# lyclyc52/Instance_NeRF

Measured on AMD Instinct MI355X. Metric: Msamples/sec (train+infer) 3D-FRONT 800x800 at 1/2/4/8 MI355X; PSNR parity, higher is better.
Workload: dtype f32; 1 GPU; render 800x800 synthetic 3D-FRONT-like room, hash-grid NeRF L=16 F=2 T=6119864 sigma+rgb (BASELINE configs[1]), one view per step per GPU; parallelism=views sharded over 1 GPU(s), no data-path collective

## Files before the change

### instance_nerf_amd/csrc/field_fused.hip

```cpp
#include <atomic>
#include <mutex>
#include <type_traits>

#include "common.h"
#include "grid_common.h"

namespace inr {

typedef float f32x4 __attribute__((ext_vector_type(4)));
typedef __bf16 bf16x8 __attribute__((ext_vector_type(8)));

#ifndef INR_MLP_FP32
#define INR_MLP_FP32 0
#endif

#ifdef INR_PROBE_BUILD
#include "probe/field_probe.h"
#else
#if defined(INR_PROBE_MODE) || defined(INR_PROBE_STATIC) || defined(INR_PROBE_SLOW_XCD)
#error "INR_PROBE_* switches need -DINR_PROBE_BUILD (tools/build_probe.py): those variants produce wrong results"
#endif
#define INR_PROBE_PROLOGUE()
#define INR_PROBE_SCHEDULE(steal)
#define INR_PROBE_TILE()
// ... 250 lines not shown
    hi[t] = __uint_as_float(r0) + __uint_as_float(r1);
  }
}


template <int N_MT, int N_G>
__device__ __forceinline__ void layer(const float4* __restrict__ w, int lane, const f32x4* in, f32x4* out) {
  if constexpr (N_MT == 1) {
    f32x4 a0 = {0.f, 0.f, 0.f, 0.f}, a1 = {0.f, 0.f, 0.f, 0.f};
#pragma unroll
    for (int g = 0; g < N_G; g += 2) {
      __builtin_amdgcn_sched_barrier(0);
      const float4 w0 = w[g * 64 + lane], w1 = w[(g + 1) * 64 + lane];
      a0 = __builtin_amdgcn_mfma_f32_16x16x4f32(w0.x, in[g][0], a0, 0, 0, 0);
      a1 = __builtin_amdgcn_mfma_f32_16x16x4f32(w1.x, in[g + 1][0], a1, 0, 0, 0);
      a0 = __builtin_amdgcn_mfma_f32_16x16x4f32(w0.y, in[g][1], a0, 0, 0, 0);
      a1 = __builtin_amdgcn_mfma_f32_16x16x4f32(w1.y, in[g + 1][1], a1, 0, 0, 0);
      a0 = __builtin_amdgcn_mfma_f32_16x16x4f32(w0.z, in[g][2], a0, 0, 0, 0);
      a1 = __builtin_amdgcn_mfma_f32_16x16x4f32(w1.z, in[g + 1][2], a1, 0, 0, 0);
      a0 = __builtin_amdgcn_mfma_f32_16x16x4f32(w0.w, in[g][3], a0, 0, 0, 0);
      a1 = __builtin_amdgcn_mfma_f32_16x16x4f32(w1.w, in[g + 1][3], a1, 0, 0, 0);
    }
    out[0] = a0 + a1;
  } else {
    f32x4 acc[N_MT];
#pragma unroll
    for (int mt = 0; mt < N_MT; ++mt) acc[mt] = f32x4{0.f, 0.f, 0.f, 0.f};
#pragma unroll
    for (int g = 0; g < N_G; ++g) {
      __builtin_amdgcn_sched_barrier(0);
      float4 wv[N_MT];
#pragma unroll
      for (int mt = 0; mt < N_MT; ++mt) wv[mt] = w[(mt * N_G + g) * 64 + lane];
#pragma unroll
      for (int mt = 0; mt < N_MT; ++mt) acc[mt] = __builtin_amdgcn_mfma_f32_16x16x4f32(wv[mt].x, in[g][0], acc[mt], 0, 0, 0);
#pragma unroll
      for (int mt = 0; mt < N_MT; ++mt) acc[mt] = __builtin_amdgcn_mfma_f32_16x16x4f32(wv[mt].y, in[g][1], acc[mt], 0, 0, 0);
#pragma unroll
      for (int mt = 0; mt < N_MT; ++mt) acc[mt] = __builtin_amdgcn_mfma_f32_16x16x4f32(wv[mt].z, in[g][2], acc[mt], 0, 0, 0);
#pragma unroll
      for (int mt = 0; mt < N_MT; ++mt) acc[mt] = __builtin_amdgcn_mfma_f32_16x16x4f32(wv[mt].w, in[g][3], acc[mt], 0, 0, 0);
    }
#pragma unroll
    for (int mt = 0; mt < N_MT; ++mt) out[mt] = acc[mt];
  }
}

struct SplitB {
  uint4 hi, lo;
};

__device__ __forceinline__ void split2(float x0, float x1, uint32_t& hi, uint32_t& lo) {
  const uint32_t u0 = __float_as_uint(x0), u1 = __float_as_uint(x1);
  hi = __builtin_amdgcn_perm(u1, u0, 0x07060302u);
  const float l0 = x0 - __uint_as_float(u0 & 0xFFFF0000u);
  const float l1 = x1 - __uint_as_float(u1 & 0xFFFF0000u);
  lo = __builtin_amdgcn_perm(__float_as_uint(l1), __float_as_uint(l0), 0x07060302u);
}
__device__ __forceinline__ SplitB split8(const f32x4 a, const f32x4 b) {
  SplitB r;
  split2(a[0], a[1], r.hi.x, r.lo.x);
  split2(a[2], a[3], r.hi.y, r.lo.y);
  split2(b[0], b[1], r.hi.z, r.lo.z);
  split2(b[2], b[3], r.hi.w, r.lo.w);
  return r;
}
__device__ __forceinline__ f32x4 mfma_bf(const uint4 a, const uint4 b, const f32x4 c) {
  return __builtin_amdgcn_mfma_f32_16x16x32_bf16(__builtin_bit_cast(bf16x8, a), __builtin_bit_cast(bf16x8, b), c, 0, 0, 0);
}

template <int N_MT, int N_S>
__device__ __forceinline__ void layer_bf(const uint4* __restrict__ w, int lane, const SplitB* in, f32x4* out) {
  if constexpr (N_MT == 1) {
    f32x4 a0 = {0.f, 0.f, 0.f, 0.f}, a1 = a0, a2 = a0;
#pragma unroll
    for (int st = 0; st < N_S; ++st) {
      __builtin_amdgcn_sched_barrier(0);
      const uint4 wh = w[(st * 2 + 0) * 64 + lane], wlo = w[(st * 2 + 1) * 64 + lane];
      a0 = mfma_bf(wh, in[st].hi, a0);
      a1 = mfma_bf(wlo, in[st].hi, a1);
      a2 = mfma_bf(wh, in[st].lo, a2);
    }
    out[0] = a0 + (a1 + a2);
  } else {
    f32x4 acc[N_MT];
#pragma unroll
    for (int mt = 0; mt < N_MT; ++mt) acc[mt] = f32x4{0.f, 0.f, 0.f, 0.f};
#pragma unroll
    for (int st = 0; st < N_S; ++st) {
      __builtin_amdgcn_sched_barrier(0);
      uint4 wh[N_MT], wlo[N_MT];
#pragma unroll
      for (int mt = 0; mt < N_MT; ++mt) {
        wh[mt] = w[((mt * N_S + st) * 2 + 0) * 64 + lane];
        wlo[mt] = w[((mt * N_S + st) * 2 + 1) * 64 + lane];
      }
#pragma unroll
      for (int mt = 0; mt < N_MT; ++mt) acc[mt] = mfma_bf(wh[mt], in[st].hi, acc[mt]);
#pragma unroll
      for (int mt = 0; mt < N_MT; ++mt) acc[mt] = mfma_bf(wlo[mt], in[st].hi, acc[mt]);
#pragma unroll
      for (int mt = 0; mt < N_MT; ++mt) acc[mt] = mfma_bf(wh[mt], in[st].lo, acc[mt]);
    }
#pragma unroll
    for (int mt = 0; mt < N_MT; ++mt) out[mt] = acc[mt];
  }
}

typedef _Float16 f16x8_t __attribute__((ext_vector_type(8)));
typedef _Float16 f16x2_t __attribute__((ext_vector_type(2)));
typedef float f32x2_t __attribute__((ext_vector_type(2)));
__device__ __forceinline__ uint32_t pack_f16x2(float a, float b) {
  const f32x2_t v = {a, b};
  return __builtin_bit_cast(uint32_t, __builtin_convertvector(v, f16x2_t));
}
template <int N_MT, int N_S>
__device__ __forceinline__ void layer_h1(const uint4* __restrict__ w, int lane, const uint4* in, f32x4* out) {
  f32x4 acc[N_MT];
#pragma unroll
  for (int mt = 0; mt < N_MT; ++mt) acc[mt] = f32x4{0.f, 0.f, 0.f, 0.f};
#pragma unroll
  for (int st = 0; st < N_S; ++st) {
    __builtin_amdgcn_sched_barrier(0);
#pragma unroll
    for (int mt = 0; mt < N_MT; ++mt)
      acc[mt] = __builtin_amdgcn_mfma_f32_16x16x32_f16(__builtin_bit_cast(f16x8_t, w[((mt * N_S + st) * 2 + 0) * 64 + lane]),
                                                       __builtin_bit_cast(f16x8_t, in[st]), acc[mt], 0, 0, 0);
  }
#pragma unroll
  for (int mt = 0; mt < N_MT; ++mt) out[mt] = acc[mt];
}

template <int N_MT, int N_G, bool kFast = false>
__device__ __forceinline__ void mlp_layer(const float4* __restrict__ wsec, int lane, const f32x4* in, f32x4* out) {
#if INR_MLP_FP32
  layer<N_MT, N_G>(wsec, lane, in, out);
#else
  if constexpr (kFast) {
    uint4 b[N_G / 2];
#pragma unroll
    for (int st = 0; st < N_G / 2; ++st)
      b[st] = uint4{pack_f16x2(in[2 * st][0], in[2 * st][1]), pack_f16x2(in[2 * st][2], in[2 * st][3]),
                    pack_f16x2(in[2 * st + 1][0], in[2 * st + 1][1]), pack_f16x2(in[2 * st + 1][2], in[2 * st + 1][3])};
    layer_h1<N_MT, N_G / 2>(reinterpret_cast<const uint4*>(wsec), lane, b, out);
  } else {
    SplitB b[N_G / 2];
#pragma unroll
    for (int st = 0; st < N_G / 2; ++st) b[st] = split8(in[2 * st], in[2 * st + 1]);
    layer_bf<N_MT, N_G / 2>(reinterpret_cast<const uint4*>(wsec), lane, b, out);
  }
#endif
}

__device__ __forceinline__ float rgb_channel_of_lane(const f32x4 o) {
  const auto a = __builtin_amdgcn_permlane16_swap(__float_as_uint(o[0]), __float_as_uint(o[1]), false, false);
  const unsigned a0 = a[0];
  const auto b = __builtin_amdgcn_permlane32_swap(a0, __float_as_uint(o[2]), false, false);
  const unsigned b0 = b[0];
  return __uint_as_float(b0);
}
__device__ __forceinline__ float sigmoid_rgb(float o) {
  return __frcp_rn(1.0f + __expf(-o));
}

__device__ __forceinline__ float select4(int q, float a, float b, float c, float d) {
  return q == 0 ? a : (q == 1 ? b : (q == 2 ? c : d));
}

struct TileIn {
  float x0, x1, x2;
  float d0, d1, d2;
  bool oob;
};

__device__ __forceinline__ float to_x01(float x, float bound, float rb, float) { return (x + bound) / rb; }

template <bool kDir>
__device__ __forceinline__ void load_tile_in(const float* __restrict__ x, const float* __restrict__ d, int64_t m,
                                             float bound, float rb, float rb_inv, TileIn& t) {
  t.x0 = to_x01(x[m * 3 + 0], bound, rb, rb_inv);
  t.x1 = to_x01(x[m * 3 + 1], bound, rb, rb_inv);
  t.x2 = to_x01(x[m * 3 + 2], bound, rb, rb_inv);
  t.oob = oob01(t.x0, t.x1, t.x2);
  if (t.oob) t.x0 = t.x1 = t.x2 = 0.0f;
  if constexpr (kDir) {
    t.d0 = d[m * 3]; t.d1 = d[m * 3 + 1]; t.d2 = d[m * 3 + 2];
  }
}

constexpr int kXcdChunkLog2 = 10;
#ifndef INR_STEAL_SHIFT
#define INR_STEAL_SHIFT 1
#endif
constexpr int kStealRoundsShift = INR_STEAL_SHIFT;
struct TileSched {
  int64_t lo, hi;
  int64_t first;
  int64_t stride;
  int64_t main_local = 0, tail_base = 0;
  int64_t n_main = 0, tail = 0;
  int64_t static_local = 0;
  uint32_t xcd = 0;
  bool interleaved = false, hybrid = false;
  __device__ __forceinline__ int64_t tile_of(int y, int64_t u) const {
    if (u < main_local) return ((((u >> kXcdChunkLog2) << 3) + y) << kXcdChunkLog2) + (u & ((1 << kXcdChunkLog2) - 1));
    return n_main + tail * y / 8 + (u - main_local);
  }
  __device__ __forceinline__ int64_t local_end(int y) const { return main_local + tail * (y + 1) / 8 - tail * y / 8; }
  __device__ __forceinline__ int64_t tile(int64_t i) const {
    if (interleaved) {
      const int64_t u = first + i * stride;
      if (u < main_local)
        return ((((u >> kXcdChunkLog2) << 3) + xcd) << kXcdChunkLog2) + (u & ((1 << kXcdChunkLog2) - 1));
      return tail_base + (u - main_local);
    }
    return first + i * stride;
  }
};
__device__ __forceinline__ TileSched make_sched(int64_t n_tiles, int waves_per_block, bool steal = false) {
  const int nb = gridDim.x, b = blockIdx.x;
  const int w = threadIdx.x >> 6;
  TileSched s;
  if (nb % 8 == 0) {
    const int xcd = b & 7, local = b >> 3, per = nb >> 3;
    const int64_t rounds = n_tiles >> (kXcdChunkLog2 + 3);
    if (rounds >= 4) {
      const int64_t n_main = rounds << (kXcdChunkLog2 + 3), tail = n_tiles - n_main;
      s.interleaved = true;
      s.xcd = (uint32_t)xcd;
      s.main_local = rounds << kXcdChunkLog2;
      s.n_main = n_main;
      s.tail = tail;
      s.hybrid = steal;
      s.static_local = steal ? (rounds - max((int64_t)1, rounds >> kStealRoundsShift)) << kXcdChunkLog2 : s.main_local;
      s.tail_base = n_main + tail * xcd / 8;
      s.lo = 0;
      s.hi = n_main + tail * (xcd + 1) / 8;
      s.first = (int64_t)local * waves_per_block + w;
      s.stride = (int64_t)per * waves_per_block;
      return s;
    }
    s.lo = n_tiles * xcd / 8;
    s.hi = n_tiles * (xcd + 1) / 8;
    s.first = s.lo + (int64_t)local * waves_per_block + w;
    s.stride = (int64_t)per * waves_per_block;
  } else {
    s.lo = 0;
    s.hi = n_tiles;
    s.first = (int64_t)b * waves_per_block + w;
    s.stride = (int64_t)nb * waves_per_block;
  }
  return s;
}

constexpr int kFieldThreads = 512;
constexpr int kGroupChunkLog2 = 6;
constexpr int kGroupDraw = 1;
constexpr int kGroupPools = 4;
struct GroupDraw {
  unsigned long long* cursor;
  int owner, n_owner;
  __device__ __forceinline__ void init(unsigned long long* cursors, int pools) {
    const int n_xcd = (gridDim.x % 8 == 0) ? 8 : 1;
    const int n_pool = (gridDim.x % (8 * pools) == 0) ? pools : 1;
    const int xcd = (n_xcd == 8) ? (int)(blockIdx.x & 7) : 0;
    const int pool = (n_pool > 1) ? (int)((blockIdx.x >> 3) % pools) : 0;
    owner = pool * n_xcd + xcd;
    n_owner = n_pool * n_xcd;
    cursor = cursors + owner;
  }
  __device__ __forceinline__ int64_t group_of(uint32_t u) const {
    const int64_t chunk = (int64_t)(u >> kGroupChunkLog2) * n_owner + owner;
    return (chunk << kGroupChunkLog2) + (u & ((1u << kGroupChunkLog2) - 1u));
  }
  __device__ __forceinline__ int64_t draw() const { return group_of((uint32_t)atomicAdd(cursor, (unsigned long long)kGroupDraw)); }
};
constexpr int kStealPools = 4, kStealOwners = 8 * kStealPools, kStealDraw = 4, kStealBlockLog2 = 6;
struct TileWalk {
  TileSched s;
  unsigned long long* cur;
  int lane, own, owner, sub;
  int64_t it, k_base;
  unsigned long long raw_next;
  bool dyn;
  __device__ __forceinline__ void init(const TileSched& sched, unsigned long long* cursors) {
    s = sched; cur = cursors; lane = threadIdx.x & 63; it = 0; dyn = false; sub = kStealDraw; k_base = 0; raw_next = 0;
    own = owner = (int)(((blockIdx.x >> 3) % kStealPools) * 8 + (blockIdx.x & 7));
    if (!cursors) s.hybrid = false;
    if (!s.hybrid) s.static_local = s.main_local;
  }
  __device__ __forceinline__ int64_t pool_len(int o) const {
    const int64_t nb = (s.local_end(o & 7) - s.static_local + (1 << kStealBlockLog2) - 1) >> kStealBlockLog2;
    const int p = o >> 3;
    return nb > p ? ((nb - p + kStealPools - 1) / kStealPools) << kStealBlockLog2 : 0;
  }
  __device__ __forceinline__ int64_t local_of(int o, int64_t k) const {
    return s.static_local + ((((k >> kStealBlockLog2) * kStealPools) + (o >> 3)) << kStealBlockLog2) +
           (k & ((1 << kStealBlockLog2) - 1));
  }
  __device__ __forceinline__ unsigned long long issue(int o) const {
    unsigned long long v = 0;
    if (lane == 0) v = atomicAdd(cur + o, (unsigned long long)kStealDraw);
    return v;
  }
  __device__ __forceinline__ static int64_t uniform(unsigned long long v) {
    return (int64_t)(((unsigned long long)(uint32_t)__builtin_amdgcn_readfirstlane((int)(v >> 32)) << 32) |
                     (uint32_t)__builtin_amdgcn_readfirstlane((int)v));
  }
  __device__ __forceinline__ int scan() const {
    bool live = false;
    if (lane < kStealOwners) live = (int64_t)__hip_atomic_load(cur + lane, __ATOMIC_RELAXED, __HIP_MEMORY_SCOPE_AGENT) < pool_len(lane);
    const uint32_t mask = (uint32_t)__ballot(live);
    for (int i = 0; i < kStealOwners; ++i) {
      const int o = (((own >> 3) + i) % kStealPools) * 8 + (((own & 7) + i / kStealPools) & 7);
      if ((mask >> o) & 1u) return o;
    }
    return -1;
  }
  __device__ __forceinline__ int64_t next() {
    if (!dyn) {
      if (!s.hybrid) {
        const int64_t t = s.tile(it++);
        return t < s.hi ? t : -1;
      }
      const int64_t u = s.first + (it++) * s.stride;
      if (u < s.static_local) return s.tile_of((int)s.xcd, u);
      dyn = true;
      raw_next = issue(owner);
    }
    for (;;) {
      if (sub < kStealDraw) {
        const int64_t u = local_of(owner, k_base + sub);
        ++sub;
        if (u < s.local_end(owner & 7)) return s.tile_of(owner & 7, u);
        continue;
      }
      int64_t k = uniform(raw_next);
      while (k >= pool_len(owner)) {
        const int o = scan();
        if (o < 0) return -1;
        owner = o;
        k = uniform(issue(owner));
      }
      k_base = k;
      sub = 0;
      raw_next = issue(owner);
    }
  }
};
constexpr int kFieldMinWaves = 2;

__device__ __forceinline__ f32x4 load4(const float* p) {
  const float4 v = *reinterpret_cast<const float4*>(p);
  return f32x4{v.x, v.y, v.z, v.w};
}
__device__ __forceinline__ void store4(float* p, f32x4 v) {
  *reinterpret_cast<float4*>(p) = make_float4(v[0], v[1], v[2], v[3]);
}
__device__ __forceinline__ f32x4 mask4(f32x4 g, f32x4 h) {
  return f32x4{h[0] > 0.f ? g[0] : 0.f, h[1] > 0.f ? g[1] : 0.f, h[2] > 0.f ? g[2] : 0.f, h[3] > 0.f ? g[3] : 0.f};
}

struct NerfSave {
  float *enc, *h1, *so, *cin, *c1, *c2;
};

template <bool kColor, bool kTable = false, int kSave = 0, bool kHalf = false, bool kFast = false, bool kPre = false>
__global__ void __launch_bounds__(kFieldThreads, kFieldMinWaves) k_nerf_fwd(const float* __restrict__ x, const float* __restrict__ d,
                                                               int64_t M, const int32_t* __restrict__ n_dev, float bound,
                                                               const float2* __restrict__ emb, uint32_t emb_bytes, GridDesc G,
                                                               const float4* __restrict__ packed, float density_scale,
                                                               float* __restrict__ sigma, float* __restrict__ rgb,
                                                               float* __restrict__ geo, const int32_t* __restrict__ ray_ids,
                                                               const float4* __restrict__ shq, NerfSave sv,
                                                               unsigned long long* __restrict__ steal) {
  extern __shared__ __attribute__((aligned(16))) float4 wl[];
  INR_PROBE_PROLOGUE();
  __builtin_amdgcn_s_setprio(3);
  constexpr int kStage = (kColor ? kNerfFloats : kCol0) / 4;
  for (int i = threadIdx.x; i < kStage; i += kFieldThreads) wl[i] = packed[i];
  LevelRec* recs = reinterpret_cast<LevelRec*>(wl + kStage);
  stage_level_recs(G, recs);
  __syncthreads();

  constexpr int kWaves = kFieldThreads / 64;
  const int lane = threadIdx.x & 63, q = lane >> 4, j = lane & 15;
  int64_t n = M;
  if (n_dev) n = min((int64_t)*n_dev, M);
  const int64_t n_tiles = (n + 15) >> 4;
  const float rb = 2.0f * bound;
  const float rb_inv = 0.0f;
  INR_PROBE_SCHEDULE(steal);
  TileWalk walk;
  walk.init(make_sched(n_tiles, kWaves, steal != nullptr), steal);

  const bool all_hashed[4] = {slot_all_hashed(G, 0), slot_all_hashed(G, 1), slot_all_hashed(G, 2), slot_all_hashed(G, 3)};
  const __amdgpu_buffer_rsrc_t rsrc = __builtin_amdgcn_make_buffer_rsrc((void*)emb, 0, (int)emb_bytes, 0x00020000);

  for (int64_t tile = walk.next(); tile >= 0; tile = walk.next()) {
    INR_PROBE_TILE();
    const int64_t m = tile * 16 + j;
    const bool valid = m < n;
    TileIn me;
    f32x4 sh_in = {0.f, 0.f, 0.f, 0.f};
    if constexpr (kTable) {
      const int64_t mm = valid ? m : n - 1;
      me.x0 = x[mm * 3 + 0]; me.x1 = x[mm * 3 + 1]; me.x2 = x[mm * 3 + 2];
      const float4 t4 = shq[(int64_t)ray_ids[mm] * 4 + q];
      sh_in = f32x4{t4.x, t4.y, t4.z, t4.w};
    } else {
      load_tile_in<kColor>(x, d, valid ? m : n - 1, bound, rb, rb_inv, me);
    }

    f32x4 enc[2];
    {
      Gathered g;
      uint32_t rec_off = (uint32_t)q * 4u * (uint32_t)sizeof(LevelRec);
      asm volatile("" : "+v"(rec_off));
      typedef float v2f __attribute__((ext_vector_type(2)));
      v2f fine_a = {0.f, 0.f}, fine_b = {0.f, 0.f};
      if constexpr (kPre) {
        static_assert(!kPre || kTable, "the sliced feed is a variant of the table feed");
        static_assert(kSliceLevels == 3, "lane map below");
        const v2f* pre = reinterpret_cast<const v2f*>(d);
        const int64_t m_pad = (M + 31) & ~(int64_t)31, mm = valid ? m : n - 1;
        const int sl = (q & 1) ? 1 : 0;
        fine_a = __builtin_nontemporal_load(pre + (int64_t)sl * m_pad + mm);
        fine_b = __builtin_nontemporal_load(pre + (int64_t)(sl + 1) * m_pad + mm);
      }
      issue_gathers<kHalf, kPre>(reinterpret_cast<const LevelRec*>(reinterpret_cast<const char*>(recs) + rec_off), all_hashed,
                                 rsrc, me.x0, me.x1, me.x2, g);
      __builtin_amdgcn_sched_barrier(0);
      blend<kHalf>(g, enc[0], enc[1]);
      if constexpr (kPre) {
        if (q == 2) enc[1] = f32x4{enc[1][0], enc[1][1], fine_a.x, fine_a.y};
        else if (q == 3) enc[1] = f32x4{fine_a.x, fine_a.y, fine_b.x, fine_b.y};
      }
    }
    if constexpr (!kTable) {
      if (me.oob) enc[0] = enc[1] = f32x4{0.f, 0.f, 0.f, 0.f};
    }
    INR_PROBE_AFTER_GATHER();

    f32x4 h1[4];
    mlp_layer<4, 2, kFast>(wl + kSig0 / 4, lane, enc, h1);
#pragma unroll
    for (int t = 0; t < 4; ++t) h1[t] = relu4(h1[t]);
    f32x4 h2[1];
    mlp_layer<1, 4, kFast>(wl + kSig1 / 4, lane, h1, h2);

    if (valid) {
      if (q == 0) sigma[m] = __expf(h2[0][0]) * density_scale;
      if (INR_PROBE_GEO_IS_OUTPUT && geo) {
#pragma unroll
        for (int r = 0; r < 4; ++r) {
          const int row = 4 * q + r;
          if (row >= 1) geo[m * 15 + row - 1] = h2[0][r];
        }
      }
    }

    if constexpr (kColor) {
      f32x4 cin[2];
      if constexpr (kTable) {
        cin[0] = sh_in;
      } else {
        float sh[16];
        sh4(me.d0, me.d1, me.d2, sh);
#pragma unroll
        for (int ks = 0; ks < 4; ++ks) cin[0][ks] = select4(q, sh[4 * ks], sh[4 * ks + 1], sh[4 * ks + 2], sh[4 * ks + 3]);
      }
      cin[1] = h2[0];
      f32x4 c1[4], c2[4], o[1];
      mlp_layer<4, 2, kFast>(wl + kCol0 / 4, lane, cin, c1);
#pragma unroll
      for (int t = 0; t < 4; ++t) c1[t] = relu4(c1[t]);
      mlp_layer<4, 4, kFast>(wl + kCol1 / 4, lane, c1, c2);
#pragma unroll
      for (int t = 0; t < 4; ++t) c2[t] = relu4(c2[t]);
      mlp_layer<1, 4, kFast>(wl + kCol2 / 4, lane, c2, o);
      if constexpr (kSave == 2) {
        if (valid) {
#pragma unroll
          for (int t = 0; t < 2; ++t) store4(sv.enc + m * 32 + 16 * t + 4 * q, enc[t]);
        }
      }
      if constexpr (kSave == 1) {
        if (valid) {
#pragma unroll
          for (int t = 0; t < 2; ++t) store4(sv.enc + m * 32 + 16 * t + 4 * q, enc[t]);
          store4(sv.so + m * 16 + 4 * q, h2[0]);
#pragma unroll
          for (int t = 0; t < 4; ++t) {
            store4(sv.h1 + m * 64 + 16 * t + 4 * q, h1[t]);
            store4(sv.c1 + m * 64 + 16 * t + 4 * q, c1[t]);
            store4(sv.c2 + m * 64 + 16 * t + 4 * q, c2[t]);
          }
#pragma unroll
          for (int ks = 0; ks < 4; ++ks) sv.cin[m * 32 + 4 * ks + q] = cin[0][ks];
#pragma unroll
          for (int r = 0; r < 4; ++r) {
            const int row = 4 * q + r;
            sv.cin[m * 32 + (row >= 1 ? 15 + row : 31)] = row >= 1 ? h2[0][r] : 0.f;
          }
        }
      }
      const float ch = sigmoid_rgb(rgb_channel_of_lane(o[0]));
      if (valid && q < 3) rgb[m * 3 + q] = ch;
    }
  }
  INR_PROBE_EPILOGUE();
}

constexpr int kSliceThreads = 256;
constexpr int kSliceTilesPerIter = 4;
struct SliceX {
  float x0, x1, x2;
};
__device__ __forceinline__ SliceX slice_load_x(const float* __restrict__ x01, int64_t m, int64_t M) {
  const int64_t mm = m < M ? m : M - 1;
  const float* p = x01 + mm * 3;
  return SliceX{__builtin_nontemporal_load(p), __builtin_nontemporal_load(p + 1), __builtin_nontemporal_load(p + 2)};
}
__global__ void __launch_bounds__(kSliceThreads) k_grid_fine_slices(const float* __restrict__ x01, int64_t M,
                                                                    const float2* __restrict__ emb, uint32_t emb_bytes,
                                                                    GridDesc G, float* __restrict__ pre) {
  const int slice = blockIdx.y;
  const int l = 16 - kSliceLevels + slice;
  const float sc = G.scales[l];
  const uint32_t m_ = G.mask[l], res1 = G.res1[l];
  const bool h = m_ != 0;
  const uint32_t base = G.offsets[l] * 8u, pa = h ? 2654435761u : res1, pb = h ? 805459861u : res1 * res1;
  const uint32_t mask = h ? m_ : 0xFFFFFFFFu;
  const __amdgpu_buffer_rsrc_t rsrc = __builtin_amdgcn_make_buffer_rsrc((void*)emb, 0, (int)emb_bytes, 0x00020000);
  const int lane = threadIdx.x & 63, w = threadIdx.x >> 6;
  const uint32_t side = (uint32_t)(lane & 1);
  constexpr int kWaves = kSliceThreads / 64;
  constexpr int kT = kSliceTilesPerIter;
  const int64_t m_pad = (M + 31) & ~(int64_t)31;
  const int64_t n_iter = (M + 32 * kT - 1) / (32 * kT);
  float* __restrict__ out = pre + (int64_t)slice * m_pad * 2;
  for (int64_t it = (int64_t)blockIdx.x * kWaves + w; it < n_iter; it += (int64_t)gridDim.x * kWaves) {
    u32x2 rows[kT][4];
    float wx[kT], fy[kT], fz[kT];
#pragma unroll
    for (int t = 0; t < kT; ++t) {
      const SliceX X = slice_load_x(x01, (it * kT + t) * 32 + (lane >> 1), M);
      const float px = X.x0 * sc + 0.5f, py = X.x1 * sc + 0.5f, pz = X.x2 * sc + 0.5f;
      const float fx = __builtin_amdgcn_fractf(px);
      wx[t] = side ? fx : 1.0f - fx;
      fy[t] = __builtin_amdgcn_fractf(py); fz[t] = __builtin_amdgcn_fractf(pz);
      const uint32_t c = (uint32_t)px + side, cy = (uint32_t)py, cz = (uint32_t)pz;
      const uint32_t hy0 = cy * pa, hy1 = hy0 + pa;
      const uint32_t hz0 = cz * pb, hz1 = hz0 + pb;
      const uint32_t yz[4] = {h ? (hy0 ^ hz0) : (hy0 + hz0), h ? (hy1 ^ hz0) : (hy1 + hz0),
                              h ? (hy0 ^ hz1) : (hy0 + hz1), h ? (hy1 ^ hz1) : (hy1 + hz1)};
#pragma unroll
      for (int k = 0; k < 4; ++k) {
        const uint32_t idx = (h ? (c ^ yz[k]) : (c + yz[k])) & mask;
        rows[t][k] = gather_row<false>(rsrc, base + idx * 8u);
      }
    }
#pragma unroll
    for (int t = 0; t < kT; ++t) {
      const f32x2 wy = {1.0f - fy[t], fy[t]};
      const f32x2 xy = wy * wx[t];
      const f32x2 w0 = xy * (1.0f - fz[t]), w1 = xy * fz[t];
      f32x2 acc = {0.f, 0.f};
      acc = __builtin_elementwise_fma(w0.xx, row2<false>(rows[t][0]), acc);
      acc = __builtin_elementwise_fma(w0.yy, row2<false>(rows[t][1]), acc);
      acc = __builtin_elementwise_fma(w1.xx, row2<false>(rows[t][2]), acc);
      acc = __builtin_elementwise_fma(w1.yy, row2<false>(rows[t][3]), acc);
      const float ox = __shfl_xor(acc.x, 1), oy = __shfl_xor(acc.y, 1);
      const float v = side ? acc.y + oy : acc.x + ox;
      const int64_t m = (it * kT + t) * 32 + (lane >> 1);
      if (m < M) __builtin_nontemporal_store(v, out + m * 2 + side);
    }
  }
}

struct LatticeDesc {
  const float* ax_w;
  const float* ax_l;
  const float* ax_h;
  int W, L, H, Wp;
};
constexpr int kMaxExtractDirs = 8;
template <bool kLattice>
__global__ void __launch_bounds__(kFieldThreads, kFieldMinWaves) k_nerf_fwd_dirs(
    const float* __restrict__ x, int64_t M, float bound, const float2* __restrict__ emb, uint32_t emb_bytes, GridDesc G,
    const float4* __restrict__ packed, const float* __restrict__ sh_dirs , int D, float4* __restrict__ out,
    LatticeDesc lat, float logit_min) {
  extern __shared__ __attribute__((aligned(16))) float4 wl[];
  constexpr int kStage = kNerfFloats / 4;
  for (int i = threadIdx.x; i < kStage; i += kFieldThreads) wl[i] = packed[i];
  LevelRec* recs = reinterpret_cast<LevelRec*>(wl + kStage);
  stage_level_recs(G, recs);
  float* shl = reinterpret_cast<float*>(recs + 16);
  for (int i = threadIdx.x; i < D * 16; i += kFieldThreads) {
    const int d = i >> 4, qq = (i >> 2) & 3, ks = i & 3;
    shl[i] = sh_dirs[d * 16 + 4 * ks + qq];
  }
  __syncthreads();
  constexpr int kWaves = kFieldThreads / 64;
  const int lane = threadIdx.x & 63, q = lane >> 4, j = lane & 15;
  const int64_t n_tiles = (M + 15) >> 4;
  const float rb = 2.0f * bound;
  const TileSched sched = make_sched(n_tiles, kWaves);
  const bool all_hashed[4] = {slot_all_hashed(G, 0), slot_all_hashed(G, 1), slot_all_hashed(G, 2), slot_all_hashed(G, 3)};
  const __amdgpu_buffer_rsrc_t rsrc = __builtin_amdgcn_make_buffer_rsrc((void*)emb, 0, (int)emb_bytes, 0x00020000);
  const float inv_d = 1.0f / (float)D;
  for (int64_t it = 0, tile = sched.tile(0); tile < sched.hi; tile = sched.tile(++it)) {
    int64_t m = tile * 16 + j;
    bool valid = m < M;
    TileIn me;
    if constexpr (kLattice) {
      const int64_t row = m / lat.Wp;
      const int iw = (int)(m - row * lat.Wp);
      const int il = (int)(row / lat.H), ih = (int)(row - (int64_t)il * lat.H);
      valid = valid && iw < lat.W;
      const int cw = min(iw, lat.W - 1), cl = min(il, lat.L - 1);
      me.x0 = to_x01(fminf(fmaxf(lat.ax_w[cw], -bound), bound), bound, rb, 0.0f);
      me.x1 = to_x01(fminf(fmaxf(lat.ax_l[cl], -bound), bound), bound, rb, 0.0f);
      me.x2 = to_x01(fminf(fmaxf(lat.ax_h[ih], -bound), bound), bound, rb, 0.0f);
      me.oob = oob01(me.x0, me.x1, me.x2);
      if (me.oob) me.x0 = me.x1 = me.x2 = 0.0f;
      m = ((int64_t)cw * lat.L + cl) * lat.H + ih;
    } else {
      load_tile_in<false>(x, nullptr, valid ? m : M - 1, bound, rb, 0.0f, me);
    }
    f32x4 enc[2];
    {
      Gathered g;
      uint32_t rec_off = (uint32_t)q * 4u * (uint32_t)sizeof(LevelRec);
      asm volatile("" : "+v"(rec_off));
      issue_gathers(reinterpret_cast<const LevelRec*>(reinterpret_cast<const char*>(recs) + rec_off), all_hashed, rsrc,
                    me.x0, me.x1, me.x2, g);
      __builtin_amdgcn_sched_barrier(0);
      blend(g, enc[0], enc[1]);
    }
    if (me.oob) enc[0] = enc[1] = f32x4{0.f, 0.f, 0.f, 0.f};
    f32x4 h1[4], h2[1];
    mlp_layer<4, 2>(wl + kSig0 / 4, lane, enc, h1);
#pragma unroll
    for (int t = 0; t < 4; ++t) h1[t] = relu4(h1[t]);
    mlp_layer<1, 4>(wl + kSig1 / 4, lane, h1, h2);
    float ch = 0.f;
    for (int d = 0; d < D; ++d) {
      f32x4 cin[2], c1[4], c2[4], o[1];
      const float4 s4 = *reinterpret_cast<const float4*>(shl + d * 16 + q * 4);
      cin[0] = f32x4{s4.x, s4.y, s4.z, s4.w};
      cin[1] = h2[0];
      mlp_layer<4, 2>(wl + kCol0 / 4, lane, cin, c1);
#pragma unroll
      for (int t = 0; t < 4; ++t) c1[t] = relu4(c1[t]);
      mlp_layer<4, 4>(wl + kCol1 / 4, lane, c1, c2);
#pragma unroll
      for (int t = 0; t < 4; ++t) c2[t] = relu4(c2[t]);
      mlp_layer<1, 4>(wl + kCol2 / 4, lane, c2, o);
      ch += sigmoid_rgb(rgb_channel_of_lane(o[0]));
    }
    if (valid) {
      float* o4 = reinterpret_cast<float*>(out + m);
      if (q < 3) o4[q] = ch * inv_d;
      if (q == 0) o4[3] = fmaxf(h2[0][0], logit_min);
    }
  }
}

template <int K_MT, int kSave = 0>
__global__ void __launch_bounds__(kFieldThreads, kFieldMinWaves) k_instance_fwd(const float* __restrict__ x, int64_t M,
                                                                   const int32_t* __restrict__ n_dev, float bound,
                                                                   const float2* __restrict__ emb, uint32_t emb_bytes,
                                                                   GridDesc G, const float4* __restrict__ packed,
                                                                   float* __restrict__ logits, float* __restrict__ enc_out,
                                                                   float* __restrict__ h1_out, float* __restrict__ h2_out) {
  extern __shared__ __attribute__((aligned(16))) float4 wl[];
  constexpr int K = K_MT * 16;
  constexpr int kStage = (kIns2 + K * 64) / 4;
  for (int i = threadIdx.x; i < kStage; i += kFieldThreads) wl[i] = packed[i];
  LevelRec* recs = reinterpret_cast<LevelRec*>(wl + kStage);
  stage_level_recs(G, recs);
  __syncthreads();

  constexpr int kWaves = kFieldThreads / 64;
  const int lane = threadIdx.x & 63, q = lane >> 4, j = lane & 15;
  int64_t n = M;
  if (n_dev) n = min((int64_t)*n_dev, M);
  const int64_t n_tiles = (n + 15) >> 4;
  const float rb = 2.0f * bound;
  const float rb_inv = 0.0f;
  const TileSched sched = make_sched(n_tiles, kWaves);

  const bool all_hashed[4] = {slot_all_hashed(G, 0), slot_all_hashed(G, 1), slot_all_hashed(G, 2), slot_all_hashed(G, 3)};
  const __amdgpu_buffer_rsrc_t rsrc = __builtin_amdgcn_make_buffer_rsrc((void*)emb, 0, (int)emb_bytes, 0x00020000);

  for (int64_t it = 0, tile = sched.tile(0); tile < sched.hi; tile = sched.tile(++it)) {
    const int64_t m = tile * 16 + j;
    const bool valid = m < n;
    TileIn me;
    load_tile_in<false>(x, nullptr, valid ? m : n - 1, bound, rb, rb_inv, me);
    f32x4 enc[2];
    {
      Gathered g;
      uint32_t rec_off = (uint32_t)q * 4u * (uint32_t)sizeof(LevelRec);
      asm volatile("" : "+v"(rec_off));
      issue_gathers(reinterpret_cast<const LevelRec*>(reinterpret_cast<const char*>(recs) + rec_off), all_hashed, rsrc,
                    me.x0, me.x1, me.x2, g);
      __builtin_amdgcn_sched_barrier(0);
      blend(g, enc[0], enc[1]);
    }
    if (me.oob) enc[0] = enc[1] = f32x4{0.f, 0.f, 0.f, 0.f};
    f32x4 h1[4], h2[4], o[K_MT];
    mlp_layer<4, 2>(wl + kIns0 / 4, lane, enc, h1);
#pragma unroll
    for (int t = 0; t < 4; ++t) h1[t] = relu4(h1[t]);
    mlp_layer<4, 4>(wl + kIns1 / 4, lane, h1, h2);
#pragma unroll
    for (int t = 0; t < 4; ++t) h2[t] = relu4(h2[t]);
    mlp_layer<K_MT, 4>(wl + kIns2 / 4, lane, h2, o);
    if (valid) {
#pragma unroll
      for (int mt = 0; mt < K_MT; ++mt) {
        float4 v = make_float4(o[mt][0], o[mt][1], o[mt][2], o[mt][3]);
        *reinterpret_cast<float4*>(logits + m * K + 16 * mt + 4 * q) = v;
      }
      if constexpr (kSave != 0) {
#pragma unroll
        for (int t = 0; t < 2; ++t)
          *reinterpret_cast<float4*>(enc_out + m * 32 + 16 * t + 4 * q) = make_float4(enc[t][0], enc[t][1], enc[t][2], enc[t][3]);
      }
      if constexpr (kSave == 1) {
#pragma unroll
        for (int t = 0; t < 4; ++t) {
          *reinterpret_cast<float4*>(h1_out + m * 64 + 16 * t + 4 * q) = make_float4(h1[t][0], h1[t][1], h1[t][2], h1[t][3]);
          *reinterpret_cast<float4*>(h2_out + m * 64 + 16 * t + 4 * q) = make_float4(h2[t][0], h2[t][1], h2[t][2], h2[t][3]);
        }
      }
    }
  }
}

constexpr uint8_t kLabelEmpty = 255;
constexpr int kNoChannel = 0x7fffffff;
template <int K_MT>
__global__ void __launch_bounds__(kFieldThreads, kFieldMinWaves) k_instance_lattice(
    LatticeDesc lat, float bound, const float2* __restrict__ emb_n, uint32_t emb_n_bytes, GridDesc Gn,
    const float4* __restrict__ packed_n, float density_scale, float sigma_thresh, const float2* __restrict__ emb_i,
    uint32_t emb_i_bytes, GridDesc Gi, const float4* __restrict__ packed_i, int K, uint8_t* __restrict__ labels,
    float* __restrict__ confidence, float* __restrict__ logit_out) {
  extern __shared__ __attribute__((aligned(16))) float4 wl[];
  constexpr int kStageN = kCol0 / 4;
  constexpr int kStageI = (kIns2 + K_MT * 16 * 64) / 4;
  const float4* wn = wl;
  const float4* wi = wl + kStageN;
  for (int i = threadIdx.x; i < kStageN; i += kFieldThreads) wl[i] = packed_n[i];
  for (int i = threadIdx.x; i < kStageI; i += kFieldThreads) wl[kStageN + i] = packed_i[i];
  LevelRec* recs_n = reinterpret_cast<LevelRec*>(wl + kStageN + kStageI);
  LevelRec* recs_i = recs_n + 16;
  stage_level_recs(Gn, recs_n);
  stage_level_recs(Gi, recs_i);
  __syncthreads();

  constexpr int kWaves = kFieldThreads / 64;
  const int lane = threadIdx.x & 63, q = lane >> 4, j = lane & 15;
  const int64_t n_tiles = ((int64_t)lat.Wp * lat.L * lat.H) >> 4;
  const float rb = 2.0f * bound;
  const TileSched sched = make_sched(n_tiles, kWaves);
  const bool hashed_n[4] = {slot_all_hashed(Gn, 0), slot_all_hashed(Gn, 1), slot_all_hashed(Gn, 2), slot_all_hashed(Gn, 3)};
  const bool hashed_i[4] = {slot_all_hashed(Gi, 0), slot_all_hashed(Gi, 1), slot_all_hashed(Gi, 2), slot_all_hashed(Gi, 3)};
  const __amdgpu_buffer_rsrc_t rsrc_n = __builtin_amdgcn_make_buffer_rsrc((void*)emb_n, 0, (int)emb_n_bytes, 0x00020000);
  const __amdgpu_buffer_rsrc_t rsrc_i = __builtin_amdgcn_make_buffer_rsrc((void*)emb_i, 0, (int)emb_i_bytes, 0x00020000);
  for (int64_t it = 0, tile = sched.tile(0); tile < sched.hi; tile = sched.tile(++it)) {
    const int64_t m = tile * 16 + j;
    const int64_t row = m / lat.Wp;
    const int iw = (int)(m - row * lat.Wp);
    const int il = (int)(row / lat.H), ih = (int)(row - (int64_t)il * lat.H);
    const bool valid = iw < lat.W;
    const int cw = min(iw, lat.W - 1);
    TileIn me;
    me.x0 = to_x01(fminf(fmaxf(lat.ax_w[cw], -bound), bound), bound, rb, 0.0f);
    me.x1 = to_x01(fminf(fmaxf(lat.ax_l[il], -bound), bound), bound, rb, 0.0f);
    me.x2 = to_x01(fminf(fmaxf(lat.ax_h[ih], -bound), bound), bound, rb, 0.0f);
    me.oob = oob01(me.x0, me.x1, me.x2);
    if (me.oob) me.x0 = me.x1 = me.x2 = 0.0f;
    const int64_t o = ((int64_t)cw * lat.L + il) * lat.H + ih;
    const uint32_t rec_off0 = (uint32_t)q * 4u * (uint32_t)sizeof(LevelRec);

    float logit;
    {
      f32x4 enc[2];
      {
        Gathered g;
        uint32_t rec_off = rec_off0;
        asm volatile("" : "+v"(rec_off));
        issue_gathers(reinterpret_cast<const LevelRec*>(reinterpret_cast<const char*>(recs_n) + rec_off), hashed_n, rsrc_n,
                      me.x0, me.x1, me.x2, g);
        __builtin_amdgcn_sched_barrier(0);
        blend(g, enc[0], enc[1]);
      }
      if (me.oob) enc[0] = enc[1] = f32x4{0.f, 0.f, 0.f, 0.f};
      f32x4 h1[4], h2[1];
      mlp_layer<4, 2>(wn + kSig0 / 4, lane, enc, h1);
#pragma unroll
      for (int t = 0; t < 4; ++t) h1[t] = relu4(h1[t]);
      mlp_layer<1, 4>(wn + kSig1 / 4, lane, h1, h2);
      logit = __shfl(h2[0][0], j);
    }
    const bool occ = valid && __expf(logit) * density_scale >= sigma_thresh;
    if (logit_out && valid && q == 0) logit_out[o] = logit;
    if (__ballot(occ) == 0) {
      if (valid && q == 0) {
        labels[o] = kLabelEmpty;
// ... 1787 lines not shown
```

Measured before the change: 6506 Msamples/s.

## Interleave bf16 split conversions of MLP activations with MFMA issue slots

Adds fused MLP layer routines that overlap the ReLU and bf16 hi/lo splitting of each output tile with the MFMAs of the next tiles, using scheduling barriers to pin the interleave. Sigma and color networks in the field forward and the table-based color path now run through these fused layers when the bf16 path is in use. The aim is to hide the VALU conversion work between layers behind matrix-core latency instead of running it as separate phases. In exchange it adds heavy manual scheduling that may raise register pressure, and the fixed barriers limit what the compiler can reorder.

```diff
diff --git a/instance_nerf_amd/csrc/field_fused.hip b/instance_nerf_amd/csrc/field_fused.hip
--- a/instance_nerf_amd/csrc/field_fused.hip
+++ b/instance_nerf_amd/csrc/field_fused.hip
@@ -426,6 +426,108 @@
 #endif
 }
 
+constexpr int kSlotFence = 0x0104;
+
+__device__ __forceinline__ void split_part(int part, bool relu, bool odd, f32x4& v, SplitB& d) {
+  if (part == 0) {
+    if (relu) v = relu4(v);
+    const uint32_t h0 = __builtin_amdgcn_perm(__float_as_uint(v[1]), __float_as_uint(v[0]), 0x07060302u);
+    const uint32_t h1 = __builtin_amdgcn_perm(__float_as_uint(v[3]), __float_as_uint(v[2]), 0x07060302u);
+    if (odd) { d.hi.z = h0; d.hi.w = h1; } else { d.hi.x = h0; d.hi.y = h1; }
+  } else {
+    const float x0 = part == 1 ? v[0] : v[2], x1 = part == 1 ? v[1] : v[3];
+    const float l0 = x0 - __uint_as_float(__float_as_uint(x0) & 0xFFFF0000u);
+    const float l1 = x1 - __uint_as_float(__float_as_uint(x1) & 0xFFFF0000u);
+    const uint32_t lo = __builtin_amdgcn_perm(__float_as_uint(l1), __float_as_uint(l0), 0x07060302u);
+    if (part == 1) { if (odd) d.lo.z = lo; else d.lo.x = lo; }
+    else { if (odd) d.lo.w = lo; else d.lo.y = lo; }
+  }
+}
+struct SplitCarry {
+  f32x4 v2, v3;
+};
+__device__ __forceinline__ void carry_slot(int slot, int prev_s, SplitCarry& c, SplitB* in) {
+  if (prev_s == 3 && slot == 0) split_part(2, true, false, c.v2, in[1]);
+  if (prev_s != 0 && slot == 1) split_part(0, true, true, c.v3, in[1]);
+  if (prev_s != 0 && slot == 2) {
+    split_part(1, true, true, c.v3, in[1]);
+    split_part(2, true, true, c.v3, in[1]);
+  }
+}
+
+template <int N_S, int PREV_S, bool kExtra>
+__device__ __forceinline__ void layer4_fused(const float4* __restrict__ wsec, int lane, SplitB* in, SplitCarry& carried,
+                                             SplitB* next, SplitCarry& out, f32x4& ev, SplitB& ed) {
+  const uint4* __restrict__ w = reinterpret_cast<const uint4*>(wsec);
+  constexpr int S = 3 * N_S;
+  f32x4 acc[4];
+#pragma unroll
+  for (int mt = 0; mt < 4; ++mt) {
+    acc[mt] = f32x4{0.f, 0.f, 0.f, 0.f};
+#pragma unroll
+    for (int st = 0; st < N_S; ++st) {
+      const uint4 wh = w[((mt * N_S + st) * 2 + 0) * 64 + lane], wlo = w[((mt * N_S + st) * 2 + 1) * 64 + lane];
+#pragma unroll
+      for (int p = 0; p < 3; ++p) {
+        const int slot = mt * S + st * 3 + p;
+        acc[mt] = mfma_bf(p == 1 ? wlo : wh, p == 2 ? in[st].lo : in[st].hi, acc[mt]);
+        if (slot < 3) carry_slot(slot, PREV_S, carried, in);
+        if (kExtra && slot < 3) split_part(slot, false, false, ev, ed);
+#pragma unroll
+        for (int k = 0; k < 3; ++k) {
+          const int u = slot - 1 - k;
+          if (u >= S && u % S == 0) {
+            const int t = u / S - 1;
+            split_part(k, true, (t & 1) != 0, acc[t], next[t >> 1]);
+          }
+        }
+        __builtin_amdgcn_sched_barrier(kSlotFence);
+      }
+    }
+  }
+  out.v2 = acc[2];
+  out.v3 = acc[3];
+}
+template <int PREV_S>
+__device__ __forceinline__ f32x4 layer1_fused(const float4* __restrict__ wsec, int lane, SplitB* in, SplitCarry& carried) {
+  const uint4* __restrict__ w = reinterpret_cast<const uint4*>(wsec);
+  f32x4 a[3];
+#pragma unroll
+  for (int p = 0; p < 3; ++p) a[p] = f32x4{0.f, 0.f, 0.f, 0.f};
+#pragma unroll
+  for (int st = 0; st < 2; ++st) {
+    const uint4 wh = w[(st * 2 + 0) * 64 + lane], wlo = w[(st * 2 + 1) * 64 + lane];
+#pragma unroll
+    for (int p = 0; p < 3; ++p) {
+      a[p] = mfma_bf(p == 1 ? wlo : wh, p == 2 ? in[st].lo : in[st].hi, a[p]);
+      if (st == 0) carry_slot(p, PREV_S, carried, in);
+      __builtin_amdgcn_sched_barrier(kSlotFence);
+    }
+  }
+  return a[0] + (a[1] + a[2]);
+}
+template <bool kExtra>
+__device__ __forceinline__ f32x4 nerf_sigma_fused(const float4* __restrict__ wl, int lane, const f32x4* enc, f32x4& sh, SplitB& cin) {
+  SplitB a[1], b[2];
+  SplitCarry none, c;
+  a[0] = split8(enc[0], enc[1]);
+  layer4_fused<1, 0, kExtra>(wl + kSig0 / 4, lane, a, none, b, c, sh, cin);
+  return layer1_fused<3>(wl + kSig1 / 4, lane, b, c);
+}
+__device__ __forceinline__ f32x4 nerf_color_fused(const float4* __restrict__ wl, int lane, SplitB& cin) {
+  SplitB a[2], b[2];
+  SplitCarry none, c0, c1;
+  f32x4 no_extra;
+  layer4_fused<1, 0, false>(wl + kCol0 / 4, lane, &cin, none, a, c0, no_extra, cin);
+  layer4_fused<2, 3, false>(wl + kCol1 / 4, lane, a, c0, b, c1, no_extra, cin);
+  return layer1_fused<6>(wl + kCol2 / 4, lane, b, c1);
+}
+#if INR_MLP_FP32
+constexpr bool kFusedLayers = false;
+#else
+constexpr bool kFusedLayers = true;
+#endif
+
 __device__ __forceinline__ float rgb_channel_of_lane(const f32x4 o) {
   const auto a = __builtin_amdgcn_permlane16_swap(__float_as_uint(o[0]), __float_as_uint(o[1]), false, false);
   const unsigned a0 = a[0];
@@ -716,25 +818,56 @@
     }
     INR_PROBE_AFTER_GATHER();
 
-    f32x4 h1[4];
-    mlp_layer<4, 2, kFast>(wl + kSig0 / 4, lane, enc, h1);
-#pragma unroll
-    for (int t = 0; t < 4; ++t) h1[t] = relu4(h1[t]);
-    f32x4 h2[1];
-    mlp_layer<1, 4, kFast>(wl + kSig1 / 4, lane, h1, h2);
-
-    if (valid) {
-      if (q == 0) sigma[m] = __expf(h2[0][0]) * density_scale;
-      if (INR_PROBE_GEO_IS_OUTPUT && geo) {
-#pragma unroll
-        for (int r = 0; r < 4; ++r) {
-          const int row = 4 * q + r;
-          if (row >= 1) geo[m * 15 + row - 1] = h2[0][r];
+    constexpr bool kFused = kFusedLayers && kSave == 0 && !kFast;
+    SplitB cinb;
+    f32x4 h1[4], h2[1];
+    if constexpr (kFused) {
+      f32x4 c0 = sh_in;
+      if constexpr (kColor && !kTable) {
+        float sh[16];
+        sh4(me.d0, me.d1, me.d2, sh);
+#pragma unroll
+        for (int ks = 0; ks < 4; ++ks) c0[ks] = select4(q, sh[4 * ks], sh[4 * ks + 1], sh[4 * ks + 2], sh[4 * ks + 3]);
+      }
+      h2[0] = nerf_sigma_fused<kColor>(wl, lane, enc, c0, cinb);
+    } else {
+      mlp_layer<4, 2, kFast>(wl + kSig0 / 4, lane, enc, h1);
+#pragma unroll
+      for (int t = 0; t < 4; ++t) h1[t] = relu4(h1[t]);
+      mlp_layer<1, 4, kFast>(wl + kSig1 / 4, lane, h1, h2);
+    }
+
+    if constexpr (!(kFused && kColor)) {
+      if (valid) {
+        if (q == 0) sigma[m] = __expf(h2[0][0]) * density_scale;
+        if (INR_PROBE_GEO_IS_OUTPUT && geo) {
+#pragma unroll
+          for (int r = 0; r < 4; ++r) {
+            const int row = 4 * q + r;
+            if (row >= 1) geo[m * 15 + row - 1] = h2[0][r];
+          }
         }
       }
     }
 
-    if constexpr (kColor) {
+    if constexpr (kColor && kFused) {
+#pragma unroll
+      for (int k = 0; k < 3; ++k) split_part(k, false, true, h2[0], cinb);
+      const float sg = __expf(h2[0][0]) * density_scale;
+      const f32x4 o = nerf_color_fused(wl, lane, cinb);
+      const float ch = sigmoid_rgb(rgb_channel_of_lane(o));
+      if (valid) {
+        if (q == 0) sigma[m] = sg;
+        if (q < 3) rgb[m * 3 + q] = ch;
+        if (INR_PROBE_GEO_IS_OUTPUT && geo) {
+#pragma unroll
+          for (int r = 0; r < 4; ++r) {
+            const int row = 4 * q + r;
+            if (row >= 1) geo[m * 15 + row - 1] = h2[0][r];
+          }
+        }
+      }
+    } else if constexpr (kColor) {
       f32x4 cin[2];
       if constexpr (kTable) {
         cin[0] = sh_in;
@@ -915,24 +1048,39 @@
     }
     if (me.oob) enc[0] = enc[1] = f32x4{0.f, 0.f, 0.f, 0.f};
     f32x4 h1[4], h2[1];
-    mlp_layer<4, 2>(wl + kSig0 / 4, lane, enc, h1);
-#pragma unroll
-    for (int t = 0; t < 4; ++t) h1[t] = relu4(h1[t]);
-    mlp_layer<1, 4>(wl + kSig1 / 4, lane, h1, h2);
+    SplitB cinb;
+    if constexpr (kFusedLayers) {
+      f32x4 unused = {0.f, 0.f, 0.f, 0.f};
+      h2[0] = nerf_sigma_fused<false>(wl, lane, enc, unused, cinb);
+#pragma unroll
+      for (int k = 0; k < 3; ++k) split_part(k, false, true, h2[0], cinb);
+    } else {
+      mlp_layer<4, 2>(wl + kSig0 / 4, lane, enc, h1);
+#pragma unroll
+      for (int t = 0; t < 4; ++t) h1[t] = relu4(h1[t]);
+      mlp_layer<1, 4>(wl + kSig1 / 4, lane, h1, h2);
+    }
     float ch = 0.f;
     for (int d = 0; d < D; ++d) {
-      f32x4 cin[2], c1[4], c2[4], o[1];
       const float4 s4 = *reinterpret_cast<const float4*>(shl + d * 16 + q * 4);
-      cin[0] = f32x4{s4.x, s4.y, s4.z, s4.w};
-      cin[1] = h2[0];
-      mlp_layer<4, 2>(wl + kCol0 / 4, lane, cin, c1);
-#pragma unroll
-      for (int t = 0; t < 4; ++t) c1[t] = relu4(c1[t]);
-      mlp_layer<4, 4>(wl + kCol1 / 4, lane, c1, c2);
-#pragma unroll
-      for (int t = 0; t < 4; ++t) c2[t] = relu4(c2[t]);
-      mlp_layer<1, 4>(wl + kCol2 / 4, lane, c2, o);
-      ch += sigmoid_rgb(rgb_channel_of_lane(o[0]));
+      if constexpr (kFusedLayers) {
+        f32x4 c0 = {s4.x, s4.y, s4.z, s4.w};
+#pragma unroll
+        for (int k = 0; k < 3; ++k) split_part(k, false, false, c0, cinb);
+        ch += sigmoid_rgb(rgb_channel_of_lane(nerf_color_fused(wl, lane, cinb)));
+      } else {
+        f32x4 cin[2], c1[4], c2[4], o[1];
+        cin[0] = f32x4{s4.x, s4.y, s4.z, s4.w};
+        cin[1] = h2[0];
+        mlp_layer<4, 2>(wl + kCol0 / 4, lane, cin, c1);
+#pragma unroll
+        for (int t = 0; t < 4; ++t) c1[t] = relu4(c1[t]);
+        mlp_layer<4, 4>(wl + kCol1 / 4, lane, c1, c2);
+#pragma unroll
+        for (int t = 0; t < 4; ++t) c2[t] = relu4(c2[t]);
+        mlp_layer<1, 4>(wl + kCol2 / 4, lane, c2, o);
+        ch += sigmoid_rgb(rgb_channel_of_lane(o[0]));
+      }
     }
     if (valid) {
       float* o4 = reinterpret_cast<float*>(out + m);
```

Result: no change. 6534 Msamples/s (median of 6 runs) (+0.4%).
